# IRMVLab/EfficientLO-Net

Hardware: AMD Instinct MI355X
Metric: frame-pairs/sec (KITTI 64x1800 range image) (higher is better)
Workload: dtype f32 (1x1 convolutions as 3 fp16-MFMA products of hi/lo-split fp32 operands, fp32 accumulate)

## Files before the change

### efficientlo-net_amd/csrc/elo_fused.hip

```cpp
#include "elo_group_device.h"
#include "elo_project_device.h"
#include <atomic>
#include <cstdlib>
#include <type_traits>

namespace elo {
namespace {

typedef float f32x4 __attribute__((ext_vector_type(4)));
typedef _Float16 half4 __attribute__((ext_vector_type(4)));
typedef _Float16 half2v __attribute__((ext_vector_type(2)));

constexpr int FUSED_BLOCK = 256;
constexpr int FUSED_WAVES = 4;
__device__ __forceinline__ int ftid() { return (int)(threadIdx.x & (FUSED_BLOCK - 1)); }

constexpr int MODE_SPLIT = 0;
constexpr int MODE_HALF = 1;
constexpr int MODE_CHECKED = 2;

__device__ unsigned long long g_range_violations;
__device__ unsigned long long g_range_snapshot;
__global__ void range_take_kernel() { g_range_snapshot = atomicExch(&g_range_violations, 0ull); }

// ... 1493 lines not shown
    const int kq = lane >> 4, i16 = lane & 15;
    const long p = first_point + (K == 16 ? r >> 4 : r >> 3);
    const bool writer = (i16 & (K - 1)) == 0 && p < total_points;
#pragma unroll
    for (int cb = 0; cb < NOUT / 16; ++cb) {
        const float q[4] = {last[cb].x * mk, last[cb].y * mk, last[cb].z * mk, last[cb].w * mk};
        float o[4];
#pragma unroll
        for (int e = 0; e < 4; ++e) {
            int v = __float_as_int(q[e]);
            v = dpp_imax_all<0xb1>(v);
            v = dpp_imax_all<0x4e>(v);
            v = dpp_imax_all<0x141>(v);
            if (K == 16) v = dpp_imax_all<0x140>(v);
            o[e] = __int_as_float(v);
        }
        if (writer) feat_store4(out, p * NOUT + cb * 16 + 4 * kq, float4{o[0], o[1], o[2], o[3]}, F16);
    }
}

template <bool F16>
__device__ __forceinline__ void rr_pool_softmax4_inwave(const float4 (&logit)[4], const ActPair &v0, const ActPair &v1, float mk, int r,
                                                        int lane, long first_point, long total_points, void *out)
{
    const int kq = lane >> 4, i16 = lane & 15;
    const long p = first_point + (r >> 2);
    const bool writer = (i16 & 3) == 3 && p < total_points;
    auto shr1 = [](float x) { return __int_as_float(__builtin_amdgcn_update_dpp(0, __float_as_int(x), 0x111, 0xf, 0xf, true)); };
    auto quad_lane = [](float x, auto sel) {
        return __int_as_float(__builtin_amdgcn_update_dpp(0, __float_as_int(x), decltype(sel)::value * 0x55, 0xf, 0xf, true));
    };
    const int j = i16 & 3;
#pragma unroll
    for (int cb = 0; cb < 4; ++cb) {
        const ActPair &xp = cb < 2 ? v0 : v1;
        const float4 val = cb % 2 == 0 ? quad_value(xp.hi.x, xp.hi.y, xp.lo.x, xp.lo.y) : quad_value(xp.hi.z, xp.hi.w, xp.lo.z, xp.lo.w);
        const float l[4] = {logit[cb].x, logit[cb].y, logit[cb].z, logit[cb].w}, v[4] = {val.x, val.y, val.z, val.w};
        float den[4], acc[4];
#pragma unroll
        for (int e = 0; e < 4; ++e) {
            const float x = mk == 1.0f ? l[e] : -1e10f;
            int m = __float_as_int(x);
            m = dpp_imax_all<0xb1>(m);
            m = dpp_imax_all<0x4e>(m);
            const float ex = exp_hw(x - __int_as_float(m)), ev = ex * v[e];
            float cd = ex, ca = ev;
#pragma unroll
            for (int step = 0; step < 3; ++step) { cd = shr1(cd) + ex; ca = shr1(ca) + ev; }
            den[e] = cd; acc[e] = ca;
        }
        typedef std::integral_constant<int, 3> L3;
        float a4[4], d4[4];
#pragma unroll
        for (int e = 0; e < 4; ++e) { a4[e] = quad_lane(acc[e], L3{}); d4[e] = quad_lane(den[e], L3{}); }
        const float aj = j == 0 ? a4[0] : j == 1 ? a4[1] : j == 2 ? a4[2] : a4[3], dj = j == 0 ? d4[0] : j == 1 ? d4[1] : j == 2 ? d4[2] : d4[3];
        const float qj = aj / dj;
        const float4 o{quad_lane(qj, std::integral_constant<int, 0>{}), quad_lane(qj, std::integral_constant<int, 1>{}),
                       quad_lane(qj, std::integral_constant<int, 2>{}), quad_lane(qj, L3{})};
        if (writer) feat_store4(out, p * 64 + cb * 16 + 4 * kq, o, F16);
    }
}

constexpr int RR_BIAS_OFF = 8192;
template <int NL>
__device__ __forceinline__ float rr_bias_request(const float *const (&b)[NL], const int (&n)[NL], int tid)
{
    int at = tid;
    const float *src = b[0];
    bool found = false;
#pragma unroll
    for (int l = 0; l < NL; ++l) {
        if (!found && at < n[l]) { src = b[l] + at; found = true; }
        at -= n[l];
    }
    return *src;
}
__device__ __forceinline__ void rr_bias_store(float *lds, int tid, int total, float v) { if (tid < total) lds[RR_BIAS_OFF + tid] = v; }

template <int FP> struct Cv1Plan {
    static constexpr int NL = 6;
    static constexpr int KP[6] = {FP, 4, 2, 0, 4, 4}, TL[6] = {1, 0, 0, 1, 0, 0}, NCB[6] = {8, 4, 4, 4, 8, 4};
};

template <int C, bool F16, int MODE = MODE_SPLIT>
__device__ __forceinline__ void cv1_rr_body(const elo_cv1_args &a, const unsigned block, const unsigned nblocks)
{
    extern __shared__ __align__(16) float lds[];
    constexpr int FP = C / 16;
    const int lane = threadIdx.x & 63, wave = __builtin_amdgcn_readfirstlane(threadIdx.x >> 6);
    const int i16 = lane & 15, kq = lane >> 4;
    uint4 *ring = reinterpret_cast<uint4 *>(lds);
    const int K = a.K, P = RR_ROWS / K;
    const long total_points = (long)a.batch * a.npoints;
    const long first_point = (long)xcd_tile(block, nblocks) * P;
    unsigned bad = 0;
    RR_STAMP(0);
    typedef RrStream<Cv1Plan<FP>, MODE> Stream;
    Stream ws{{a.cv0.w_packed, a.cv1.w_packed, a.cv2.w_packed, a.cv_xyz.w_packed, a.sum_cv0.w_packed, a.sum_cv1.w_packed}, ring, wave, lane, {}};
    constexpr int E0 = Stream::first(1), E1 = Stream::first(2), E2 = Stream::first(3), E3 = Stream::first(4), E4 = Stream::first(5);
    auto fetch = [&](int g, RrW &dst) { ws.fetch(g, dst); };
    auto advance = [&](int S) { ws.advance(S); };
    ws.start();
    float4 bias[2];
#pragma unroll
    for (int t = 0; t < 2; ++t) bias[t] = *reinterpret_cast<const float4 *>(a.cv0.bias + t * 16 + 4 * kq);
    const float *const bsrc[6] = {a.cv0.bias, a.cv1.bias, a.cv2.bias, a.cv_xyz.bias, a.sum_cv0.bias, a.sum_cv1.bias};
    constexpr int BN[6] = {128, 64, 64, 64, 128, 64}, B1 = 128, B2 = 192, B3 = 256, B4 = 320, B5 = 448;
    const float bias_word = rr_bias_request(bsrc, BN, (int)threadIdx.x);
    const float *bt = lds + RR_BIAS_OFF;
    const int r = wave * 16 + i16, pi = small_div(r, K);
    long pt = first_point + pi;
    const bool used = pi < P && pt < total_points;
    if (!used) pt = first_point;
    const long gr = used ? pt * K + (r - pi * K) : first_point * K;
    const int id0 = a.idx[gr * 3 + 0], id1 = a.idx[gr * 3 + 1], id2 = a.idx[gr * 3 + 2];
    float mk = a.mask[gr];
    const int cell = (id0 * a.H2 + id1) * a.W2 + id2;
    if (!used) mk = 0.0f;
    const bool keep2 = used && mk != 0.0f;
    ActPair in0[FP];
    uint4 geo;
    {
        typedef typename std::conditional<F16, uint2, float4>::type Item;
        Item f1[FP], f2[FP];
        const Item *r1 = reinterpret_cast<const Item *>(a.feat1) + (pt * C >> 2) + kq;
        const Item *r2 = reinterpret_cast<const Item *>(a.feat2) + ((long)cell * C >> 2) + kq;
#pragma unroll
        for (int j = 0; j < FP; ++j) { f1[j] = r1[j * 4]; f2[j] = r2[j * 4]; }
        const float *c = a.xyz1 + pt * 3, *g = a.xyz2 + (long)cell * 3;
        const float pc0 = c[0], pc1 = c[1], pc2 = c[2], pg0 = g[0], pg1 = g[1], pg2 = g[2];
        ws.prime();
        auto quad = [&](const Item &v, bool keep) {
            const uint4 z{0u, 0u, 0u, 0u};
            if constexpr (F16) return keep ? quad_of_halves(v) : z;
            else return keep ? pack_quad<MODE>(v, bad) : z;
        };
#pragma unroll
        for (int j = 0; j < FP; ++j) put_quad(in0[j / 2], j % 2, quad(f1[j], used));
#pragma unroll
        for (int j = 0; j < FP; ++j) put_quad(in0[(FP + j) / 2], (FP + j) % 2, quad(f2[j], keep2));
        const float g0 = pg0 * mk, g1 = pg1 * mk, g2 = pg2 * mk;
        const float d0 = g0 - pc0, d1 = g1 - pc1, d2 = g2 - pc2;
        const float e = sqrtf(d0 * d0 + d1 * d1 + d2 * d2 + 1e-20f);
        const float4 q4 = kq == 0 ? float4{pc0, pc1, pc2, g0} : kq == 1 ? float4{g1, g2, d0, d1}
                        : kq == 2 ? float4{d2, e, 0.0f, 0.0f} : float4{0.0f, 0.0f, 0.0f, 0.0f};
        geo = used ? pack_quad<MODE>(q4, bad) : uint4{0u, 0u, 0u, 0u};
    }
    rr_bias_store(lds, (int)threadIdx.x, 512, bias_word);
    RR_STAMP(1);
    rr_barrier();
    RR_LAYER_STAMP(2);
    const uint4 none{0u, 0u, 0u, 0u};
    ActPair h128[4];
    auto emit0 = [&](int pass, int t, const f32x4 acc) { put_quad(h128[pass], t, pack_quad<MODE>(relu4(acc, a.cv0.relu), bad)); };
    rr_layer<FP, true, 8, 0, MODE, (F16 ? ~0u : 0u)>(in0, geo, bt, bt + B1, bias, fetch, advance, emit0);
    RR_LAYER_STAMP(3);
    ActPair h64[2];
    rr_layer<4, false, 4, E0, MODE>(h128, none, bt + B1, bt + B2, bias, fetch, advance, [&](int pass, int t, const f32x4 acc) {
        put_quad(h64[pass], t, pack_quad<MODE>(relu4(acc, a.cv1.relu), bad));
    });
    RR_LAYER_STAMP(4);
    ActPair xe[4];
    rr_layer<2, false, 4, E1, MODE>(h64, none, bt + B2, bt + B3, bias, fetch, advance, [&](int pass, int t, const f32x4 acc) {
        put_quad(xe[pass], t, pack_quad<MODE>(relu4(acc, a.cv2.relu), bad));
    });
    RR_LAYER_STAMP(5);
    {
        ActPair unused[1];
        rr_layer<0, true, 4, E2, MODE>(unused, geo, bt + B3, bt + B4, bias, fetch, advance, [&](int pass, int t, const f32x4 acc) {
            put_quad(xe[2 + pass], t, pack_quad<MODE>(relu4(acc, a.cv_xyz.relu), bad));
        });
    }
    RR_LAYER_STAMP(6);
    rr_layer<4, false, 8, E3, MODE>(xe, none, bt + B4, bt + B5, bias, fetch, advance, [&](int pass, int t, const f32x4 acc) {
        put_quad(h128[pass], t, pack_quad<MODE>(relu4(acc, a.sum_cv0.relu), bad));
    });
    RR_LAYER_STAMP(7);
    float4 logit[4];
    rr_layer<4, false, 4, E4, MODE>(h128, none, bt + B5, nullptr, bias, fetch, advance, [&](int pass, int t, const f32x4 acc) {
        logit[2 * pass + t] = relu4(acc, a.sum_cv1.relu);
    });
    RR_STAMP(8);
    rr_pool<F16>(lds, logit, xe[0], xe[1], mk, r, wave, lane, K, P, first_point, total_points, a.out);
    RR_STAMP(9);
    report_violations<MODE>(bad, a.range_counter);
}

template <int C, bool F16, int MODE = MODE_SPLIT>
__global__ __launch_bounds__(RR_WAVES * 64, 4) void cv1_rr_kernel(const elo_cv1_args a)
{
    cv1_rr_body<C, F16, MODE>(a, blockIdx.x, gridDim.x);
}
template <int C> struct Cv2Plan {
    static constexpr int NL = 3;
    static constexpr int KP[3] = {0, 4 + C / 32, 4}, TL[3] = {1, C == 16 ? 1 : 0, 0}, NCB[3] = {4, 8, 4};
};

template <int C, bool F16, int MODE = MODE_SPLIT>
__global__ __launch_bounds__(RR_WAVES * 64, 4) void cv2_rr_kernel(const elo_cv2_args a)
{
    extern __shared__ __align__(16) float lds[];
// ... 308 lines not shown
        for (int j = 0; j < 2; ++j) {
            if (!live[j]) continue;
            const int pp = (wave * 16) / K + j, b = pb[j];
            const float cx = pc[j][0], cy = pc[j][1], cz = pc[j][2];
            auto emit = [&](int slot, int hw) {
                cell_row[pp * K + slot] = (b * a.H2 + (hw >> 16)) * a.W2 + (hw & 0xffff);
                mask_row[pp * K + slot] = 1.0f;
            };
            int count = 0;
            if (!(pick_max(sq3(cx, cy, cz), ELO_EPS) <= ELO_EPS)) {
                const GridBuf gb = grid_buffer(a.src_xyz + (size_t)b * a.H2 * a.W2 * 3);
                count = wave_random_k_prefetched(gb, a.H2, a.W2, KT, K, lds_off, ph[j], pw[j], cx, cy, cz, r2, first[j], emit);
            }
            if (count + lane < K) { cell_row[pp * K + count + lane] = 0; mask_row[pp * K + count + lane] = 0.0f; }
        }
    }
    RR_STAMP(2);
    __syncthreads();
    RR_STAMP(3);
    const int r = wave * 16 + i16, pi = small_div(r, K);
    const int cell = cell_row[r];
    const bool used = cell >= 0;
    const float mk = mask_row[r];
    const float c0 = cxyz[(pi < P ? pi : 0) * 3 + 0], c1 = cxyz[(pi < P ? pi : 0) * 3 + 1], c2 = cxyz[(pi < P ? pi : 0) * 3 + 2];
    ActPair in0[FPB / 2];
    uint4 dxyz;
    const bool keep = used && mk != 0.0f;
    {
        typedef typename std::conditional<F16, uint2, float4>::type Item;
        Item f[FPB];
        const long cc = used ? cell : 0;
        const Item *rf = reinterpret_cast<const Item *>(a.src_feat) + (cc * C >> 2) + kq;
#pragma unroll
        for (int j = 0; j < FPB; ++j) f[j] = rf[j * 4];
        const float *g = a.src_xyz + cc * 3;
        const float x = g[0], y = g[1], z = g[2];
        ws.prime();
        auto quad = [&](const Item &v) {
            const uint4 zq{0u, 0u, 0u, 0u};
            if constexpr (F16) return keep ? quad_of_halves(v) : zq;
            else return keep ? pack_quad<MODE>(v, bad) : zq;
        };
#pragma unroll
        for (int j = 0; j < FPB; ++j) put_quad(in0[j / 2], j % 2, quad(f[j]));
        const float4 d = kq == 0 ? float4{x * mk - c0, y * mk - c1, z * mk - c2, 0.0f} : float4{0.0f, 0.0f, 0.0f, 0.0f};
        dxyz = used ? pack_quad<MODE>(d, bad) : uint4{0u, 0u, 0u, 0u};
    }
    rr_bias_store(lds, tid, N1 + N2 + N3, bias_word);
    RR_STAMP(4);
    rr_barrier();
    RR_STAMP(5);
    const uint4 none{0u, 0u, 0u, 0u};
    ActPair h1[N1 / 32];
    auto emit0 = [&](int pass, int t, const f32x4 acc) { put_quad(h1[pass], t, pack_quad<MODE>(relu4(acc, a.layers[0].relu), bad)); };
    rr_layer<FPB / 2, true, N1 / 16, 0, MODE, (F16 ? ~0u : 0u)>(in0, dxyz, bt, bt + B1, bias, fetch, advance, emit0);
    RR_STAMP(6);
    float4 last[NOUT / 16];
    if constexpr (N3 == 0) {
        rr_layer<N1 / 32, false, N2 / 16, E0, MODE>(h1, none, bt + B1, nullptr, bias, fetch, advance, [&](int pass, int t, const f32x4 acc) {
            last[2 * pass + t] = relu4(acc, a.layers[1].relu);
        });
    } else {
        ActPair h2[N2 / 32];
        rr_layer<N1 / 32, false, N2 / 16, E0, MODE>(h1, none, bt + B1, bt + B2, bias, fetch, advance, [&](int pass, int t, const f32x4 acc) {
            put_quad(h2[pass], t, pack_quad<MODE>(relu4(acc, a.layers[1].relu), bad));
        });
        rr_layer<N2 / 32, false, NOUT / 16, E1, MODE>(h2, none, bt + B2, nullptr, bias, fetch, advance, [&](int pass, int t, const f32x4 acc) {
            last[2 * pass + t] = relu4(acc, a.layers[2].relu);
        });
    }
    RR_STAMP(7);
    if ((K == 8 || K == 16) && a.layers[N3 ? 2 : 1].relu) rr_pool_max_inwave<NOUT, F16>(last, mk, r, lane, K, first_point, total_points, a.out);
    else rr_pool_max<NOUT, F16>(lds, last, mk, r, wave, lane, K, P, first_point, total_points, a.out);
    RR_STAMP(8);
    report_violations<MODE>(bad, a.range_counter);
}

template <int FPB, int N1, int N2, int N3, bool F16, int MODE = MODE_SPLIT>
__global__ __launch_bounds__(RR_WAVES * 64, 4) void setconv_rr_kernel(const JobPair<elo_setconv_args> jobs)
{
    setconv_rr_body<FPB, N1, N2, N3, F16, MODE>(jobs.job[blockIdx.y], blockIdx.x, gridDim.x);
}

template <int C, bool F16, int MODE>
__global__ __launch_bounds__(RR_WAVES * 64, 4) void cv1_setconv_rr_kernel(const elo_cv1_args a, const JobPair<elo_setconv_args> jobs,
                                                                         const unsigned n_cv, const unsigned n_sc)
{
    if (blockIdx.x < n_cv) {
        cv1_rr_body<C, F16, MODE>(a, blockIdx.x, n_cv);
    } else {
        const unsigned r = blockIdx.x - n_cv, j = r >= n_sc ? 1u : 0u;
        setconv_rr_body<4, 128, 64, 0, F16, MODE>(jobs.job[j], j ? r - n_sc : r, n_sc);
    }
}
template <int CIN, int N1, int N2, int N3, int MODE>
__global__ __launch_bounds__(ELO_BLOCK, 2) void setconv_narrow_kernel(const elo_setconv_args a)
{
    constexpr int G = 32, PER_BLOCK = ELO_BLOCK / G, C = CIN - 3, CB3 = N3 / 16;
    static_assert((C == 16 || C == 3) && N1 <= 16 && N2 <= 16 && (N3 == 16 || N3 == 32), "the pyramid's two narrow set-conv layers");
    __shared__ int slot_hw[PER_BLOCK][G];
    const int tid = threadIdx.x;
    const int l64 = tid & 63, i16 = l64 & 15, kq = l64 >> 4;
    unsigned bad = 0, wbad = 0;
    auto wq = [&](const elo_dense &L, const int LK, const int LN, int k0, int n) {
        const int nc = n < LN ? n : LN - 1;
        float v[4];
#pragma unroll
        for (int e = 0; e < 4; ++e) {
            const int k = k0 + e < LK ? k0 + e : LK - 1;
            v[e] = L.w_plain[k * LN + nc];
        }
#pragma unroll
        for (int e = 0; e < 4; ++e) v[e] = (k0 + e < LK && n < LN) ? v[e] : 0.0f;
        return float4{v[0], v[1], v[2], v[3]};
    };
    auto bq = [&](const elo_dense &L, const int LN, int n0) {
        float v[4];
#pragma unroll
        for (int e = 0; e < 4; ++e) v[e] = L.bias[n0 + e < LN ? n0 + e : LN - 1];
#pragma unroll
        for (int e = 0; e < 4; ++e) v[e] = n0 + e < LN ? v[e] : 0.0f;
        return float4{v[0], v[1], v[2], v[3]};
    };
    const float4 w1a = wq(a.layers[0], CIN, N1, 4 * kq, i16), w1b = C == 16 ? wq(a.layers[0], CIN, N1, 16 + 4 * kq, i16) : float4{0.0f, 0.0f, 0.0f, 0.0f};
    const float4 w2f = wq(a.layers[1], N1, N2, 4 * kq, i16);
    float4 w3f[CB3];
#pragma unroll
    for (int cb = 0; cb < CB3; ++cb) w3f[cb] = wq(a.layers[2], N2, N3, 4 * kq, cb * 16 + i16);
    const float4 b1 = bq(a.layers[0], N1, 4 * kq), b2 = bq(a.layers[1], N2, 4 * kq);
    float4 b3[CB3];
#pragma unroll
    for (int cb = 0; cb < CB3; ++cb) b3[cb] = bq(a.layers[2], N3, cb * 16 + 4 * kq);

    const int g = tid / G, lane = tid % G, shift = (tid & 63) / G * G;
    const elo_group_spec &gs = a.group;
    const int KT = gs.kernel_h * gs.kernel_w, kW = gs.kernel_w, hh = gs.kernel_h / 2, hw2 = gs.kernel_w / 2;
    int off[SMALL_STEPS];
    const int *order = gs.decoded_hw ? gs.decoded_hw : gs.random_hw;
#pragma unroll
    for (int st = 0; st < SMALL_STEPS; ++st) off[st] = order[st * G + lane < KT ? st * G + lane : 0];
    const long total = (long)a.batch * a.npoints;
    const long first = (long)xcd_tile(blockIdx.x, gridDim.x) * PER_BLOCK;
    const long pt = first + g;
    const bool live = pt < total;
    const long ptc = live ? pt : total - 1;
    int b, n, hc, wc;
    split_point(ptc, a.npoints, b, n);
    if (a.centre_hw) {
        const int2 c2 = reinterpret_cast<const int2 *>(a.centre_hw)[ptc];
        hc = c2.x; wc = c2.y;
    } else { hc = n / a.W; wc = n - hc * a.W; }
    if (!gs.decoded_hw) {
#pragma unroll
        for (int st = 0; st < SMALL_STEPS; ++st) off[st] = ((off[st] / kW - hh) << 16) | ((off[st] % kW - hw2) & 0xffff);
    }
    const float *cp = a.xyz1_grid + (((long)b * a.H + hc) * a.W + wc) * 3;
    const float cx = cp[0], cy = cp[1], cz = cp[2];
    const float *grid2 = a.src_xyz + (size_t)b * a.H2 * a.W2 * 3;
    const int base_h = div_stride(hc, gs.stride_h), base_w = div_stride(wc, gs.stride_w);
    RawSlot raw[SMALL_STEPS];
#pragma unroll
    for (int st = 0; st < SMALL_STEPS; ++st) raw[st] = fetch_slot(grid2, a.H2, a.W2, off[st], base_h, base_w, st * G + lane < KT);
    if (live && lane < 3 && a.new_xyz) a.new_xyz[pt * 3 + lane] = lane == 0 ? cx : lane == 1 ? cy : cz;
    const float r2 = gs.distance * gs.distance;
    slot_hw[g][lane] = -1;
    int taken = 0;
    const bool centre_ok = !(pick_max(sq3(cx, cy, cz), ELO_EPS) <= ELO_EPS);
#pragma unroll
    for (int st = 0; st < SMALL_STEPS; ++st) {
        if (st > 0 && (st * G >= KT || __builtin_amdgcn_ballot_w64(taken < G) == 0)) break;
        const Probe pr = judge(raw[st], cx, cy, cz, r2);
        const bool hit = pr.hit && centre_ok && taken < G;
// ... 790 lines not shown
        const int P = RR_ROWS / a->K;
        const dim3 grid((unsigned)(((long)a->batch * a->npoints + P - 1) / P));
        const size_t lds = RR_LDS_BYTES;
        hipStream_t s = (hipStream_t)stream;
        const bool f16 = a->feat_dtype == ELO_F16;
        static_assert(RR_LDS_BYTES <= 64 * 1024, "dynamic LDS within the default limit");
#define RR(CC)                                                                                                      \
        do {                                                                                                        \
            if (f16 && plan.mode == MODE_HALF) hipLaunchKernelGGL((cv1_rr_kernel<CC, true, MODE_HALF>), grid, dim3(RR_WAVES * 64), lds, s, *a);          \
            else if (f16) hipLaunchKernelGGL((cv1_rr_kernel<CC, true, MODE_SPLIT>), grid, dim3(RR_WAVES * 64), lds, s, *a);          \
            else if (plan.mode == MODE_HALF) hipLaunchKernelGGL((cv1_rr_kernel<CC, false, MODE_HALF>), grid, dim3(RR_WAVES * 64), lds, s, *a);             \
            else hipLaunchKernelGGL((cv1_rr_kernel<CC, false, MODE_SPLIT>), grid, dim3(RR_WAVES * 64), lds, s, *a);             \
        } while (0)
        if (a->C == 16) RR(16);
        else if (a->C == 32) RR(32);
        else RR(64);
#undef RR
        ++g_rr_launches[0];
        return check_launch(who);
    }
#endif
    const dim3 grid((unsigned)plan.units);
    const size_t lds = plan.lds;
    const int S = plan.S;
    hipStream_t s = (hipStream_t)stream;
#define CALL(k) hipLaunchKernelGGL(k, grid, dim3(FUSED_BLOCK), lds, s, *a, S)
    if (a->group.random_hw) ELO_PICK(cv1_kernel, plan.t16, plan.mode, CALL);
    else ELO_PICK(cv1_meta_kernel, plan.t16, plan.mode, CALL);
#undef CALL
    return check_launch(who);
}


extern "C" int elo_cv_stage1_setconv_fused(const elo_cv1_args *a, const elo_setconv_args *ja, const elo_setconv_args *jb,
                                           elo_stream_t stream)
{
    const char *who = "elo_cv_stage1_setconv_fused";
    TilePlan pc, ps;
    if (int rc = plan_cv1(a, &pc, who)) return rc;
    if (int rc = check_setconv(ja, who)) return rc;
    if (jb) {
        if (int rc = check_setconv(jb, who)) return rc;
        if (!same_shape(ja, jb)) return fail(ELO_ERR_ARG, "%s: the two set-conv jobs must have the same shape", who);
    }
    if (int rc = plan_setconv(ja, jb, &ps, who)) return rc;
    if (ps.mode != pc.mode) return fail(ELO_ERR_ARG, "%s: the cost volume and the set-conv jobs must share one products mode", who);
    if ((long)a->batch * a->npoints == 0 || (long)ja->batch * ja->npoints == 0)
        return fail(ELO_ERR_ARG, "%s: empty batch (call the separate entry points)", who);
    SideJobs side;
    side.job[0] = *ja;
    side.job[1] = jb ? *jb : *ja;
    side.njobs = jb ? 2 : 1;
    side.S = ps.S;
    side.blocks_per_job = (int)ps.units;
    const unsigned n_cv = (unsigned)pc.units;
    const dim3 grid(n_cv + (unsigned)(ps.units * side.njobs));
    const size_t lds = pc.lds > ps.lds ? pc.lds : ps.lds;
    const int S = pc.S;
    hipStream_t s = (hipStream_t)stream;
#define CALL_T(M) do {                                                                                                  \
        if (pc.t16 && ps.t16) hipLaunchKernelGGL((cv1_setconv_kernel<16, 16, M>), grid, dim3(FUSED_BLOCK), lds, s, *a, S, n_cv, side);      \
        else if (pc.t16) hipLaunchKernelGGL((cv1_setconv_kernel<16, 32, M>), grid, dim3(FUSED_BLOCK), lds, s, *a, S, n_cv, side);           \
        else if (ps.t16) hipLaunchKernelGGL((cv1_setconv_kernel<32, 16, M>), grid, dim3(FUSED_BLOCK), lds, s, *a, S, n_cv, side);           \
        else hipLaunchKernelGGL((cv1_setconv_kernel<32, 32, M>), grid, dim3(FUSED_BLOCK), lds, s, *a, S, n_cv, side);                        \
    } while (0)
    ELO_PICK_MODE(pc.mode, CALL_T);
#undef CALL_T
    return check_launch(who);
}

static int chain_pair_form(const elo_cv1_args *a, const elo_setconv_args *ja, const elo_setconv_args *jb, int *mode_out, const char *who)
{
#ifdef ELO_DENSE_F32
    (void)a; (void)ja; (void)jb; (void)mode_out; (void)who;
    return 0;
#else
    if (!a || !ja || !jb) return 0;
    int mode = 0, mode_sc = 0, mode_sb = 0;
    if (products_mode(who, &mode, a->cv0, a->cv1, a->cv2, a->cv_xyz, a->sum_cv0, a->sum_cv1)) return 0;
    if (ja->n_layers != 2 || jb->n_layers != 2 || products_mode(who, &mode_sc, ja->layers, 2) || products_mode(who, &mode_sb, jb->layers, 2)) return 0;
    if (mode != mode_sc || mode != mode_sb || !same_shape(ja, jb) || ja->feat_dtype != a->feat_dtype) return 0;
    if (!cv_chain(a->C, mode) || setconv_chain_shape(ja, jb, mode) != 1) return 0;
    if (a->K <= 0 || a->K > 32) return 0;
    *mode_out = mode;
    return 1;
#endif
}

extern "C" int elo_cv_stage1_setconv_chain_form(const elo_cv1_args *a, const elo_setconv_args *ja, const elo_setconv_args *jb)
{
    int mode = 0;
    return chain_pair_form(a, ja, jb, &mode, "elo_cv_stage1_setconv_chain_form");
}

extern "C" int elo_cv_stage1_setconv_chain(const elo_cv1_args *a, const elo_setconv_args *ja, const elo_setconv_args *jb,
                                           elo_stream_t stream)
{
    const char *who = "elo_cv_stage1_setconv_chain";
#ifdef ELO_DENSE_F32
    (void)a; (void)ja; (void)jb; (void)stream;
    return fail(ELO_ERR_LIMIT, "%s: the fp32-MFMA comparison build has no register-resident kernels", who);
#else
    TilePlan pc, ps;
    if (int rc = plan_cv1(a, &pc, who)) return rc;
    ELO_REQUIRE(jb, who, "two set-conv jobs");
    if (int rc = check_setconv(ja, who)) return rc;
    if (int rc = check_setconv(jb, who)) return rc;
    if (!same_shape(ja, jb)) return fail(ELO_ERR_ARG, "%s: the two set-conv jobs must have the same shape", who);
    if (int rc = plan_setconv(ja, jb, &ps, who)) return rc;
    if (a->group.random_hw || !a->idx || !a->mask) return fail(ELO_ERR_ARG, "%s: the cost volume comes pre-grouped (idx / mask of the select-k pre-pass)", who);
    int mode = 0;
    if (!chain_pair_form(a, ja, jb, &mode, who) || mode != pc.mode || mode != ps.mode)
        return fail(ELO_ERR_ARG, "%s: not a chain-form launch (elo_cv_stage1_setconv_chain_form returns 0)", who);
    const long pts_cv = (long)a->batch * a->npoints, pts_sc = (long)ja->batch * ja->npoints;
    if (pts_cv == 0 || pts_sc == 0) return fail(ELO_ERR_ARG, "%s: empty batch (call the separate entry points)", who);
    const int Pc = RR_ROWS / a->K, Ps = RR_ROWS / ja->K;
    const unsigned n_cv = (unsigned)((pts_cv + Pc - 1) / Pc), n_sc = (unsigned)((pts_sc + Ps - 1) / Ps);
    const dim3 grid(n_cv + 2u * n_sc);
    JobPair<elo_setconv_args> pair;
    pair.job[0] = *ja;
    pair.job[1] = *jb;
    hipStream_t s = (hipStream_t)stream;
    const bool f16 = a->feat_dtype == ELO_F16;
#define RRP(CC)                                                                                                                              \
    do {                                                                                                                                    \
        if (f16 && mode == MODE_HALF) hipLaunchKernelGGL((cv1_setconv_rr_kernel<CC, true, MODE_HALF>), grid, dim3(RR_WAVES * 64), RR_LDS_BYTES, s, *a, pair, n_cv, n_sc);   \
        else if (f16) hipLaunchKernelGGL((cv1_setconv_rr_kernel<CC, true, MODE_SPLIT>), grid, dim3(RR_WAVES * 64), RR_LDS_BYTES, s, *a, pair, n_cv, n_sc);                 \
        else if (mode == MODE_HALF) hipLaunchKernelGGL((cv1_setconv_rr_kernel<CC, false, MODE_HALF>), grid, dim3(RR_WAVES * 64), RR_LDS_BYTES, s, *a, pair, n_cv, n_sc);   \
        else hipLaunchKernelGGL((cv1_setconv_rr_kernel<CC, false, MODE_SPLIT>), grid, dim3(RR_WAVES * 64), RR_LDS_BYTES, s, *a, pair, n_cv, n_sc);                          \
    } while (0)
    if (a->C == 16) RRP(16);
    else if (a->C == 32) RRP(32);
    else RRP(64);
#undef RRP
    ++g_rr_launches[0];
    ++g_rr_launches[2];
    ++g_chain_pair_launches;
    return check_launch(who);
#endif
}

static int plan_cv2(const elo_cv2_args *a, TilePlan *p, const char *who)
{
    ELO_REQUIRE(a, who, "null argument block");
    ELO_REQUIRE(a->batch >= 0 && a->npoints > 0 && a->K > 0 && a->H > 0 && a->W > 0 && a->C > 0, who, "bad sizes");
    ELO_REQUIRE(a->npoints == a->H * a->W, who, "npoints must equal H*W (every pixel is a centre)");
    if (a->K > 32) return fail(ELO_ERR_LIMIT, "%s: K = %d exceeds the 32-row tile", who, a->K);
    if (a->C > 64) return fail(ELO_ERR_LIMIT, "%s: C = %d exceeds 64", who, a->C);
    ELO_REQUIRE(a->xyz1 && a->feat1 && a->cost && a->out, who, "null tensor pointer");
    ELO_REQUIRE(a->group.random_hw || (a->idx && a->mask), who, "neither idx/mask nor a grouping spec");
    if (int rc = check_dtype(a->feat_dtype, who)) return rc;
    if (int rc = check_cv_features(who, a->C, a->feat_dtype == ELO_F16, {a->feat1, a->cost})) return rc;
    if (int rc = check_dense(a->xyz_enc, 10, 64, who, "sum_xyz_encoding")) return rc;
    if (int rc = check_dense(a->sum_cost0, 128 + a->C, 128, who, "sum_cost_volume_0")) return rc;
    if (int rc = check_dense(a->sum_cost1, 128, 64, who, "sum_cost_volume_1")) return rc;
    const long points = (long)a->batch * a->npoints;
    if (points >= 0x7fffffffL) return fail(ELO_ERR_LIMIT, "%s: batch * npoints beyond 2^31", who);
    p->units = 0;
    if (points == 0) return ELO_OK;
    p->S = row_stride(208);
    const int P32 = 32 / a->K, P16 = a->K <= 16 ? 16 / a->K : 1;
    const long u32 = (points + P32 - 1) / P32, u16 = (points + P16 - 1) / P16;
    if (int rc = products_mode(who, &p->mode, a->xyz_enc, a->sum_cost0, a->sum_cost1)) return rc;
    p->t16 = small_tile(u32, a->K);
    p->units = p->t16 ? u16 : u32;
    const int KT = a->group.random_hw ? a->group.kernel_h * a->group.kernel_w : 0;
    p->lds = tile_lds_bytes(p->t16 ? 16 : 32, p->S, KT, false);
    return check_group(a->group, a->H, a->W, p->lds, who);
}

extern "C" int elo_cv_stage2_fused(const elo_cv2_args *a, elo_stream_t stream)
{
    const char *who = "elo_cv_stage2_fused";
    TilePlan plan;
    if (int rc = plan_cv2(a, &plan, who)) return rc;
    if (plan.units == 0) return ELO_OK;
    const int S = plan.S, mode = plan.mode;
    const bool t16 = plan.t16;
    const size_t lds = plan.lds;
    hipStream_t s = (hipStream_t)stream;
#ifndef ELO_DENSE_F32
    if (!a->group.random_hw && cv_chain(a->C, mode)) {
        const int P = RR_ROWS / a->K;
        const dim3 rgrid((unsigned)(((long)a->batch * a->npoints + P - 1) / P));
        const bool f16 = a->feat_dtype == ELO_F16;
#define RR(CC)                                                                                                           \
        do {                                                                                                             \
            if (f16 && mode == MODE_HALF) hipLaunchKernelGGL((cv2_rr_kernel<CC, true, MODE_HALF>), rgrid, dim3(RR_WAVES * 64), RR_LDS_BYTES, s, *a);     \
            else if (f16) hipLaunchKernelGGL((cv2_rr_kernel<CC, true, MODE_SPLIT>), rgrid, dim3(RR_WAVES * 64), RR_LDS_BYTES, s, *a);     \
            else if (mode == MODE_HALF) hipLaunchKernelGGL((cv2_rr_kernel<CC, false, MODE_HALF>), rgrid, dim3(RR_WAVES * 64), RR_LDS_BYTES, s, *a);        \
            else hipLaunchKernelGGL((cv2_rr_kernel<CC, false, MODE_SPLIT>), rgrid, dim3(RR_WAVES * 64), RR_LDS_BYTES, s, *a);        \
        } while (0)
        if (a->C == 16) RR(16);
        else if (a->C == 32) RR(32);
        else RR(64);
#undef RR
        ++g_rr_launches[1];
        return check_launch(who);
    }
#endif
    const dim3 grid((unsigned)plan.units);
#define CALL(k) hipLaunchKernelGGL(k, grid, dim3(FUSED_BLOCK), lds, s, *a, S)
    ELO_PICK(cv2_kernel, t16, mode, CALL);
#undef CALL
    return check_launch(who);
}

static int upconv_ride_plan(const elo_cv2_args *a, const elo_mlp_args *ja, const elo_mlp_args *jb, TilePlan *pc, MlpPlan *pm,
                            const char *who)
{
    if (int rc = plan_cv2(a, pc, who)) return rc;
    ELO_REQUIRE(ja && jb, who, "two set-upconv jobs");
    if (int rc = plan_mlp(ja, jb, pm, who)) return rc;
    if (pc->units == 0 || ja->rows == 0) return fail(ELO_ERR_ARG, "%s: empty cost volume or jobs (call the separate entry points)", who);
    for (const elo_mlp_args *j : {ja, jb})
        if (j->n_layers2 != 0 || j->clear_scratch || j->sv_scratch)
// ... 46 lines not shown
```

### efficientlo-net_amd/fused.py

```python
import ctypes
import os

import torch

from . import _lib as L
from . import tf_util, tuning


def fp32_mfma():
    return bool(L.lib().elo_dense_f32())


PRODUCTS_SPLIT, PRODUCTS_HALF = 0, 1
_products = PRODUCTS_SPLIT


def products_mode():
    return _products


class products:

    def __init__(self, mode):
        self.mode = {"split": PRODUCTS_SPLIT, "half": PRODUCTS_HALF, PRODUCTS_SPLIT: PRODUCTS_SPLIT,
# ... 292 lines not shown

def _mlp2_args(sources, layers, before, after, layers2):
    a, out, keep = _mlp_args(sources, layers)
    rows = out.shape[0]
    before, after = _features(before, after, out)[0][:2]
    flat = lambda t: None if t is None else t.reshape(rows, t.shape[-1])
    before, after = flat(before), flat(after)
    out2 = torch.empty((rows, layers2[-1].N), dtype=out.dtype, device=out.device)
    a.n_layers2, a.layers2, a.out2 = len(layers2), _chain(layers2), out2.data_ptr()
    a.before, a.w_before = (before.data_ptr(), before.shape[1]) if before is not None else (None, 0)
    a.after, a.w_after = (after.data_ptr(), after.shape[1]) if after is not None else (None, 0)
    return a, out, out2, (keep, before, after, layers2)


def mlp2_pair(job_a, job_b, clear=None, sv=None):
    a, out_a, out2_a, _ka = _mlp2_args(**job_a)
    b, out_b, out2_b, _kb = _mlp2_args(**job_b)
    if _ride_sv(a, b, sv, out_a.dtype) or sv is None:
        _ride_clear(a, clear, out_a.dtype)
    L.call2("elo_mlp_fused2", a, b, out_a)
    lead = job_a["sources"][0].shape[:-1]
    shape = lambda t: t.reshape(lead + (t.shape[-1],))
    return (shape(out_a), shape(out2_a)), (shape(out_b), shape(out2_b))


THROUGHPUT_BATCH = 4


def _prepass_rows(stage=1, batch=1):
    e = tuning.get("cv_prepass")
    if e is None:
        return 8192 if batch >= THROUGHPUT_BATCH else (20000 if stage == 1 else 65536)
    return (1 << 60) if e == 0 else 0 if e == 1 else int(e)


_HW = {}


def _all_pixels(B, H, W, device):
    key = (B, H, W, str(device))
    hit = _HW.get(key)
    if hit is None:
        hh = torch.arange(H, dtype=torch.int32, device=device).view(1, H, 1, 1).expand(B, H, W, 1)
        ww = torch.arange(W, dtype=torch.int32, device=device).view(1, 1, W, 1).expand(B, H, W, 1)
        hit = torch.cat([hh, ww], -1).reshape(B, H * W, 2).contiguous()
        if hit.is_cuda and torch.cuda.is_current_stream_capturing():
            return hit
        if len(_HW) >= 64:
            _HW.clear()
        _HW[key] = hit
    return hit




def group_prepass(kind, xyz1_grid, xyz2_grid, group, K):
    B, H, W, _ = xyz1_grid.shape
    _, H2, W2, _ = xyz2_grid.shape
    N, kH, kW = H * W, group.kernel_h, group.kernel_w
    idx = torch.empty((B, N, K, 3), dtype=torch.int32, device=xyz1_grid.device)
    mask = torch.empty((B, N, K), dtype=torch.float32, device=xyz1_grid.device)
    if kind == "select":
        from .fused_conv import _select_dense_fits
        dense = -(-W // 64) * H * B >= tuning.get("select_dense_tiles") and _select_dense_fits(kH, kW, K, 0, group.stride_h, group.stride_w)
        entry = "elo_fused_conv_select_k_dense" if dense else "elo_fused_conv_select_k"
    else:
        RH, RW = 1 // group.stride_h + kH, 63 // group.stride_w + kW
        dense = 4 * ((kH * kW + 7) & ~7) + 16 * RH * RW + 4 * (129 * K + 256) <= 64 * 1024
        entry = "elo_fused_conv_random_k_dense" if dense else "elo_fused_conv_random_k"
    hw = None if dense else _all_pixels(B, H, W, xyz1_grid.device)
    a = L.GroupArgs(B, H, W, H2, W2, N, kH, kW, K, 0, group.distance, group.stride_h, group.stride_w,
                    xyz1_grid.data_ptr(), xyz2_grid.data_ptr(), None if dense else hw.data_ptr(), group.random_hw.data_ptr(),
                    idx.data_ptr(), None, None, mask.data_ptr())
    L.call(entry, a, idx)
    return idx, mask


def _rr_path(group, B, N, K, C, stage=1):
    return (group is not None and not group.want_indices and K <= 32 and B * N * K >= _prepass_rows(stage, B)
            and group.stride_h == 1 and group.stride_w == 1 and not fp32_mfma()
            and C in (16, 32, 64))


_RECORD = None


class recording:

    def __enter__(self):
        global _RECORD
        self.prev, _RECORD = _RECORD, []
        return _RECORD

    def __exit__(self, *exc):
        global _RECORD
        _RECORD = self.prev


def _record(stage, args, kwargs):
    keep = lambda v: v.detach().clone() if torch.is_tensor(v) else v
    kw = {k: keep(v) for k, v in kwargs.items() if k != "side"}
    if kwargs.get("group") is not None:
        g = kwargs["group"]
        kw["group"] = Grouping(g.random_hw.clone(), [g.kernel_h, g.kernel_w], g.distance, g.stride_h, g.stride_w)
    _RECORD.append((stage, tuple(keep(v) for v in args), kw, bool(kwargs.get("side"))))


def cv_stage1(xyz1, feat1, xyz2_proj, feat2_proj, idx, mask, cv0, cv1, cv2, cv_xyz, sum_cv0, sum_cv1, group=None, K=None,
              side=None, side_chain=False):
    L.require_gpu(xyz1, feat1, xyz2_proj, feat2_proj, idx, mask)
    if _RECORD is not None:
        _record(1, (xyz1, feat1, xyz2_proj, feat2_proj, idx, mask, cv0, cv1, cv2, cv_xyz, sum_cv0, sum_cv1), dict(group=group, K=K, side=side))
    xyz1, xyz2_proj = _f32c(xyz1), _f32c(xyz2_proj)
    (feat1, feat2_proj), dt, code = _features(feat1, feat2_proj)
    _, H2, W2, C = feat2_proj.shape
    B, N = xyz1.shape[0], xyz1.shape[1]
    ptr = lambda x: x.data_ptr() if x is not None else None
    chain_jobs = None
    if side and side_chain:
        rr = len(side) == 2 and N == H2 * W2 and _rr_path(group, B, N, K, C)
        if rr:
            chain_jobs = [_setconv_args(**job) for job in side]
            probe = L.Cv1Args(B, N, K, H2, W2, C, None, None, None, None, None, None, cv0.struct(), cv1.struct(), cv2.struct(),
                              cv_xyz.struct(), sum_cv0.struct(), sum_cv1.struct(), None, _NO_GROUP, code)
            if L.lib().elo_cv_stage1_setconv_chain_form(ctypes.byref(probe), ctypes.byref(chain_jobs[0][0]), ctypes.byref(chain_jobs[1][0])) != 1:
                chain_jobs = None
        if chain_jobs is None:
            return cv_stage1_alone(xyz1, feat1, xyz2_proj, feat2_proj, idx, mask, cv0, cv1, cv2, cv_xyz, sum_cv0, sum_cv1, group, K), None
    if (not side or chain_jobs) and N == H2 * W2 and _rr_path(group, B, N, K, C):
        idx, mask = group_prepass("select", xyz1.reshape(B, H2, W2, 3), xyz2_proj, group, K)
        group = None
    if group is None:
        idx, mask = idx.contiguous(), _f32c(mask)
        K = idx.shape[2]
    out = torch.empty((B, N, 64), dtype=dt, device=xyz1.device)
    a = L.Cv1Args(B, N, K, H2, W2, C, xyz1.data_ptr(), feat1.data_ptr(), xyz2_proj.data_ptr(), feat2_proj.data_ptr(),
                  ptr(idx), ptr(mask), cv0.struct(), cv1.struct(), cv2.struct(), cv_xyz.struct(),
                  sum_cv0.struct(), sum_cv1.struct(), out.data_ptr(),
                  group.struct(B, N, K, xyz1.device) if group is not None else _NO_GROUP, code)
    if chain_jobs:
        L.call3("elo_cv_stage1_setconv_chain", a, chain_jobs[0][0], chain_jobs[1][0], out)
        return out, [(j[1], j[2]) for j in chain_jobs]
    if side:
        jobs = [_setconv_args(**job) for job in side]
        L.call3("elo_cv_stage1_setconv_fused", a, jobs[0][0], jobs[1][0] if len(jobs) > 1 else None, out)
        return out, [(j[1], j[2]) for j in jobs]
    L.call("elo_cv_stage1_fused", a, out)
    return out


def cv_stage1_alone(xyz1, feat1, xyz2_proj, feat2_proj, idx, mask, cv0, cv1, cv2, cv_xyz, sum_cv0, sum_cv1, group, K):
    global _RECORD
    keep, _RECORD = _RECORD, None
    try:
        return cv_stage1(xyz1, feat1, xyz2_proj, feat2_proj, idx, mask, cv0, cv1, cv2, cv_xyz, sum_cv0, sum_cv1, group=group, K=K)
    finally:
        _RECORD = keep


def cv_stage2(xyz1_proj, feat1_proj, cost_proj, idx, mask, xyz_enc, sum_cost0, sum_cost1, group=None, K=None, side=None):
    L.require_gpu(xyz1_proj, feat1_proj, cost_proj, idx, mask)
    if _RECORD is not None:
        _record(2, (xyz1_proj, feat1_proj, cost_proj, idx, mask, xyz_enc, sum_cost0, sum_cost1), dict(group=group, K=K, side=side))
    xyz1_proj = _f32c(xyz1_proj)
    (feat1_proj, cost_proj), dt, code = _features(feat1_proj, cost_proj)
    B, H, W, C = feat1_proj.shape
    N = H * W
    ptr = lambda x: x.data_ptr() if x is not None else None
    if _rr_path(group, B, N, K, C, stage=2):
        idx, mask = group_prepass("random", xyz1_proj, xyz1_proj, group, K)
        group = None
    if group is None:
        idx, mask = idx.contiguous(), _f32c(mask)
        K = idx.shape[2]
    out = torch.empty((B, N, 64), dtype=dt, device=xyz1_proj.device)
    a = L.Cv2Args(B, N, K, H, W, C, xyz1_proj.data_ptr(), feat1_proj.data_ptr(), cost_proj.data_ptr(), ptr(idx),
                  ptr(mask), xyz_enc.struct(), sum_cost0.struct(), sum_cost1.struct(), out.data_ptr(),
                  group.struct(B, N, K, xyz1_proj.device) if group is not None else _NO_GROUP, code)
    if side:
        if B < THROUGHPUT_BATCH:
            jobs = [_mlp_args(**job) for job in side]
            if L.lib().elo_cv_stage2_upconv_form(ctypes.byref(a), ctypes.byref(jobs[0][0]), ctypes.byref(jobs[1][0])) == 1:
                L.call3("elo_cv_stage2_upconv_fused", a, jobs[0][0], jobs[1][0], out)
                return out, [j[1].reshape(job["sources"][0].shape[:-1] + (j[1].shape[-1],)) for j, job in zip(jobs, side)]
        L.call("elo_cv_stage2_fused", a, out)
        return out, None
    L.call("elo_cv_stage2_fused", a, out)
    return out
```

### efficientlo-net_amd/tuning.py

```python
import contextlib
import hashlib
import json
import os

def _prepass(spec):
    return None if spec in (None, "") else int(spec)


_HOST = {
    "fused": ("ELO_FUSED", lambda v: v != "0", True),
    "cv_prepass": ("ELO_CV_PREPASS", _prepass, None),
    "select_dense_tiles": ("ELO_SELECT_DENSE_TILES", int, 1024),
    "merge_points": ("ELO_MERGE_POINTS", int, 8192),
    "merge_level_points": ("ELO_MERGE_LEVEL_POINTS", int, 2000),
    "chain_pair": ("ELO_CHAIN_PAIR", lambda v: v != "0", True),
    "native_submit": ("ELO_NATIVE_SUBMIT", lambda v: v != "0", True),
    "sv_ride": ("ELO_SV_RIDE", lambda v: v != "0", True),
    "upconv_ride": ("ELO_UPCONV_RIDE", lambda v: v != "0", True),
    "train_kernels": ("ELO_TRAIN_KERNELS", lambda v: v != "0", True),
    "train_dense": ("ELO_TRAIN_DENSE", lambda v: v != "0", True),
    "train_dense_rows": ("ELO_TRAIN_DENSE_ROWS", int, 25000),
    "train_siamese_batch": ("ELO_TRAIN_SIAMESE_BATCH", lambda v: v != "0", True),
    "train_dense_fused_dz": ("ELO_TRAIN_DENSE_FUSED_DZ", lambda v: v != "0", True),
    "train_dense_dx_rows": ("ELO_TRAIN_DENSE_DX_ROWS", int, 100000),
}
_LIB = {
    "chain_forms": ("ELO_CV1_RR", 1), "narrow_mfma": ("ELO_SETCONV_NARROW_MFMA", 1), "range_check": ("ELO_RANGE_CHECK", 0),
    "select_dense_waves": ("ELO_SELECT_DENSE_WAVES", 0), "random_dense_rows": ("ELO_DENSE_ROWS", 0),
    "setconv_chain_rows": ("ELO_SETCONV_RR_ROWS", -1), "mlp_chain_rows": ("ELO_MLP_RR_ROWS", -1), "small_tile_units": ("ELO_SMALL_TILE_UNITS", 64),
    "pool_wave": ("ELO_POOL_WAVE", 1),
}


_LIB_BOOLEAN = ("chain_forms", "narrow_mfma", "range_check", "pool_wave")


def _host_from_env():
    out = {}
    for name, (var, parse, default) in _HOST.items():
        raw = os.environ.get(var)
        out[name] = default if raw is None else parse(raw)
    return out


def lib_from_env():
    out = {}
    for name, (var, _default) in _LIB.items():
        raw = os.environ.get(var)
        if raw is not None:
            value = int(raw)
            out[name] = (1 if value else 0) if name in _LIB_BOOLEAN else value
    return out


_host = _host_from_env()
_version = 0


def version():
    return _version


def bump():
    global _version
    _version += 1


def get(name):
    return _host[name]


def set_host(name, value):
    if name not in _HOST:
        raise KeyError(name)
    prev, _host[name] = _host[name], value
    bump()
    return prev


@contextlib.contextmanager
def override(**fields):
    from . import _lib
    host = {k: v for k, v in fields.items() if k in _HOST}
    lib = {k: v for k, v in fields.items() if k in _LIB}
    unknown = set(fields) - set(host) - set(lib)
    if unknown:
        raise KeyError("unknown tuning field(s): %s" % sorted(unknown))
    prev_host = {k: _host[k] for k in host}
    prev_lib = _lib.get_tuning_base() if lib else None
    try:
        _host.update(host)
        bump()
        if lib:
            _lib.set_tuning(**lib)
        yield
    finally:
        _host.update(prev_host)
        bump()
        if prev_lib is not None:
            _lib.set_tuning(**prev_lib)
# ... 17 lines not shown
```

Baseline: 12670.

## Fuse select-k grouping into the cost-volume chain kernel instead of a pre-pass

Adds an in-kernel select-k grouping stage to the cv1 chain kernel. Each block computes neighbor cells and masks into LDS scratch rather than reading idx/mask written by a separate group pre-pass kernel. This drops one kernel launch and the global round trip of idx/mask. In exchange it adds a barrier and serial per-wave selection work at the start of each cost-volume block, which may lengthen the kernel or raise register/LDS pressure.

```diff
diff --git a/efficientlo-net_amd/csrc/elo_cv1_rr_group.h b/efficientlo-net_amd/csrc/elo_cv1_rr_group.h
--- /dev/null
+++ b/efficientlo-net_amd/csrc/elo_cv1_rr_group.h
@@ -0,0 +1,57 @@
+#pragma once
+
+constexpr int CV1_RR_GROUP_OFF = 4096;
+static_assert(CV1_RR_GROUP_OFF + ((512 + 3) & ~3) + 6 * RR_ROWS + RR_WAVES * 128 <= RR_BIAS_OFF, "select-k scratch in front of the bias table");
+
+__device__ __forceinline__ void cv1_rr_group(const elo_cv1_args &a, float *lds, int P, int K, long first_point, long total_points,
+                                             int wave, int lane)
+{
+    const int tid = threadIdx.x;
+    const int KT = a.group.kernel_h * a.group.kernel_w;
+    int *lds_off = reinterpret_cast<int *>(lds + CV1_RR_GROUP_OFF);
+    int *cell_row = lds_off + ((KT + 3) & ~3);
+    float *mask_row = reinterpret_cast<float *>(cell_row + RR_ROWS);
+    int *chw = reinterpret_cast<int *>(mask_row + RR_ROWS);
+    float *cxyz = reinterpret_cast<float *>(chw + RR_ROWS);
+    unsigned *scratch = reinterpret_cast<unsigned *>(cxyz + 3 * RR_ROWS);
+    if (tid < RR_ROWS) { cell_row[tid] = -1; mask_row[tid] = 0.0f; }
+    if (tid < P) {
+        const long pt = first_point + tid;
+        const long pq = pt < total_points ? pt : first_point;
+        const int b = (int)((unsigned)pq / (unsigned)a.npoints), n = (int)((unsigned)pq - (unsigned)b * (unsigned)a.npoints);
+        const int hc = n / a.W2, wc = n - hc * a.W2;
+        const float *c = a.xyz1 + (((long)b * a.H2 + hc) * a.W2 + wc) * 3;
+        const float cx = c[0], cy = c[1], cz = c[2];
+        if (pt < total_points) { chw[tid] = (hc << 16) | wc; cxyz[tid * 3 + 0] = cx; cxyz[tid * 3 + 1] = cy; cxyz[tid * 3 + 2] = cz; }
+    }
+    stage_offsets(lds_off, a.group.random_hw, a.group.kernel_h, a.group.kernel_w, a.group.decoded_hw);
+    const float r2 = a.group.distance * a.group.distance;
+    auto uniform = [](float v) { return __int_as_float(__builtin_amdgcn_readfirstlane(__float_as_int(v))); };
+    for (int pi = wave; pi < P; pi += RR_WAVES) {
+        const long pt = first_point + pi;
+        if (pt >= total_points) break;
+        const int b = (int)((unsigned)pt / (unsigned)a.npoints);
+        const int hwc = __builtin_amdgcn_readfirstlane(chw[pi]), hc = hwc >> 16, wc = hwc & 0xffff;
+        const float cx = uniform(cxyz[pi * 3 + 0]), cy = uniform(cxyz[pi * 3 + 1]), cz = uniform(cxyz[pi * 3 + 2]);
+        auto emit = [&](int slot, int hw) {
+            cell_row[pi * K + slot] = (b * a.H2 + (hw >> 16)) * a.W2 + (hw & 0xffff);
+            mask_row[pi * K + slot] = 1.0f;
+        };
+        int count = 0;
+        if (!(pick_max(sq3(cx, cy, cz), ELO_EPS) <= ELO_EPS)) {
+            const GridBuf gb = grid_buffer(a.xyz2 + (size_t)b * a.H2 * a.W2 * 3);
+            unsigned *mine = scratch + (size_t)wave * 128;
+            count = wave_select_k(gb, a.H2, a.W2, KT, K, lds_off, div_stride(hc, a.group.stride_h), div_stride(wc, a.group.stride_w),
+                                  cx, cy, cz, r2, mine, reinterpret_cast<int *>(mine) + KT, emit);
+        }
+        for (int k = count + lane; k < K; k += 64) { cell_row[pi * K + k] = 0; mask_row[pi * K + k] = 0.0f; }
+    }
+    rr_barrier();
+}
+
+static bool cv1_rr_select_ok(const elo_cv1_args *a)
+{
+    const int KT = a->group.kernel_h * a->group.kernel_w;
+    return a->group.random_hw && !a->group.idx_out && !a->group.mask_out && a->npoints == a->H2 * a->W2 && KT > 0 && KT <= 512 &&
+           select_in_registers(KT, a->K) && a->group.stride_h > 0 && a->group.stride_w > 0;
+}
diff --git a/efficientlo-net_amd/csrc/elo_fused.hip b/efficientlo-net_amd/csrc/elo_fused.hip
--- a/efficientlo-net_amd/csrc/elo_fused.hip
+++ b/efficientlo-net_amd/csrc/elo_fused.hip
@@ -1599,7 +1599,9 @@
     static constexpr int KP[6] = {FP, 4, 2, 0, 4, 4}, TL[6] = {1, 0, 0, 1, 0, 0}, NCB[6] = {8, 4, 4, 4, 8, 4};
 };
 
-template <int C, bool F16, int MODE = MODE_SPLIT>
+#include "elo_cv1_rr_group.h"
+
+template <int C, bool F16, int MODE = MODE_SPLIT, bool GROUP = false>
 __device__ __forceinline__ void cv1_rr_body(const elo_cv1_args &a, const unsigned block, const unsigned nblocks)
 {
     extern __shared__ __align__(16) float lds[];
@@ -1629,11 +1631,19 @@
     long pt = first_point + pi;
     const bool used = pi < P && pt < total_points;
     if (!used) pt = first_point;
-    const long gr = used ? pt * K + (r - pi * K) : first_point * K;
-    const int id0 = a.idx[gr * 3 + 0], id1 = a.idx[gr * 3 + 1], id2 = a.idx[gr * 3 + 2];
-    float mk = a.mask[gr];
-    const int cell = (id0 * a.H2 + id1) * a.W2 + id2;
-    if (!used) mk = 0.0f;
+    int cell; float mk;
+    if constexpr (GROUP) {
+        cv1_rr_group(a, lds, P, K, first_point, total_points, wave, lane);
+        const int *cell_row = reinterpret_cast<const int *>(lds + CV1_RR_GROUP_OFF) + ((a.group.kernel_h * a.group.kernel_w + 3) & ~3);
+        cell = used ? cell_row[r] : 0;
+        mk = used ? reinterpret_cast<const float *>(cell_row + RR_ROWS)[r] : 0.0f;
+    } else {
+        const long gr = used ? pt * K + (r - pi * K) : first_point * K;
+        const int id0 = a.idx[gr * 3 + 0], id1 = a.idx[gr * 3 + 1], id2 = a.idx[gr * 3 + 2];
+        mk = a.mask[gr];
+        cell = (id0 * a.H2 + id1) * a.W2 + id2;
+        if (!used) mk = 0.0f;
+    }
     const bool keep2 = used && mk != 0.0f;
     ActPair in0[FP];
     uint4 geo;
@@ -2108,12 +2118,12 @@
     setconv_rr_body<FPB, N1, N2, N3, F16, MODE>(jobs.job[blockIdx.y], blockIdx.x, gridDim.x);
 }
 
-template <int C, bool F16, int MODE>
+template <int C, bool F16, int MODE, bool GROUP = false>
 __global__ __launch_bounds__(RR_WAVES * 64, 4) void cv1_setconv_rr_kernel(const elo_cv1_args a, const JobPair<elo_setconv_args> jobs,
                                                                          const unsigned n_cv, const unsigned n_sc)
 {
     if (blockIdx.x < n_cv) {
-        cv1_rr_body<C, F16, MODE>(a, blockIdx.x, n_cv);
+        cv1_rr_body<C, F16, MODE, GROUP>(a, blockIdx.x, n_cv);
     } else {
         const unsigned r = blockIdx.x - n_cv, j = r >= n_sc ? 1u : 0u;
         setconv_rr_body<4, 128, 64, 0, F16, MODE>(jobs.job[j], j ? r - n_sc : r, n_sc);
@@ -3070,6 +3080,7 @@
     if (mode != mode_sc || mode != mode_sb || !same_shape(ja, jb) || ja->feat_dtype != a->feat_dtype) return 0;
     if (!cv_chain(a->C, mode) || setconv_chain_shape(ja, jb, mode) != 1) return 0;
     if (a->K <= 0 || a->K > 32) return 0;
+    if (a->group.random_hw && !cv1_rr_select_ok(a)) return 0;
     *mode_out = mode;
     return 1;
 #endif
@@ -3096,7 +3107,9 @@
     if (int rc = check_setconv(jb, who)) return rc;
     if (!same_shape(ja, jb)) return fail(ELO_ERR_ARG, "%s: the two set-conv jobs must have the same shape", who);
     if (int rc = plan_setconv(ja, jb, &ps, who)) return rc;
-    if (a->group.random_hw || !a->idx || !a->mask) return fail(ELO_ERR_ARG, "%s: the cost volume comes pre-grouped (idx / mask of the select-k pre-pass)", who);
+    const bool group = a->group.random_hw != nullptr;
+    if (group ? !cv1_rr_select_ok(a) : (!a->idx || !a->mask))
+        return fail(ELO_ERR_ARG, "%s: neither idx / mask of the select-k pre-pass nor a grouping spec the in-kernel select-k takes", who);
     int mode = 0;
     if (!chain_pair_form(a, ja, jb, &mode, who) || mode != pc.mode || mode != ps.mode)
         return fail(ELO_ERR_ARG, "%s: not a chain-form launch (elo_cv_stage1_setconv_chain_form returns 0)", who);
@@ -3110,16 +3123,15 @@
     pair.job[1] = *jb;
     hipStream_t s = (hipStream_t)stream;
     const bool f16 = a->feat_dtype == ELO_F16;
-#define RRP(CC)                                                                                                                              \
+#define RRP(CC, G)                                                                                                                           \
     do {                                                                                                                                    \
-        if (f16 && mode == MODE_HALF) hipLaunchKernelGGL((cv1_setconv_rr_kernel<CC, true, MODE_HALF>), grid, dim3(RR_WAVES * 64), RR_LDS_BYTES, s, *a, pair, n_cv, n_sc);   \
-        else if (f16) hipLaunchKernelGGL((cv1_setconv_rr_kernel<CC, true, MODE_SPLIT>), grid, dim3(RR_WAVES * 64), RR_LDS_BYTES, s, *a, pair, n_cv, n_sc);                 \
-        else if (mode == MODE_HALF) hipLaunchKernelGGL((cv1_setconv_rr_kernel<CC, false, MODE_HALF>), grid, dim3(RR_WAVES * 64), RR_LDS_BYTES, s, *a, pair, n_cv, n_sc);   \
-        else hipLaunchKernelGGL((cv1_setconv_rr_kernel<CC, false, MODE_SPLIT>), grid, dim3(RR_WAVES * 64), RR_LDS_BYTES, s, *a, pair, n_cv, n_sc);                          \
+        if (f16 && mode == MODE_HALF) hipLaunchKernelGGL((cv1_setconv_rr_kernel<CC, true, MODE_HALF, G>), grid, dim3(RR_WAVES * 64), RR_LDS_BYTES, s, *a, pair, n_cv, n_sc);   \
+        else if (f16) hipLaunchKernelGGL((cv1_setconv_rr_kernel<CC, true, MODE_SPLIT, G>), grid, dim3(RR_WAVES * 64), RR_LDS_BYTES, s, *a, pair, n_cv, n_sc);                 \
+        else if (mode == MODE_HALF) hipLaunchKernelGGL((cv1_setconv_rr_kernel<CC, false, MODE_HALF, G>), grid, dim3(RR_WAVES * 64), RR_LDS_BYTES, s, *a, pair, n_cv, n_sc);   \
+        else hipLaunchKernelGGL((cv1_setconv_rr_kernel<CC, false, MODE_SPLIT, G>), grid, dim3(RR_WAVES * 64), RR_LDS_BYTES, s, *a, pair, n_cv, n_sc);                          \
     } while (0)
-    if (a->C == 16) RRP(16);
-    else if (a->C == 32) RRP(32);
-    else RRP(64);
+    if (a->C == 16) { if (group) RRP(16, true); else RRP(16, false); } else if (a->C == 32) { if (group) RRP(32, true); else RRP(32, false); }
+    else { if (group) RRP(64, true); else RRP(64, false); }
 #undef RRP
     ++g_rr_launches[0];
     ++g_rr_launches[2];
diff --git a/efficientlo-net_amd/fused.py b/efficientlo-net_amd/fused.py
--- a/efficientlo-net_amd/fused.py
+++ b/efficientlo-net_amd/fused.py
@@ -398,6 +398,11 @@
             and C in (16, 32, 64))
 
 
+def _rr_select(group, K):
+    KT = group.kernel_h * group.kernel_w
+    return bool(tuning.get("cv_rr_select")) and KT <= 512 and (K <= 8 or (KT <= 192 and K <= 32))
+
+
 _RECORD = None
 
 
@@ -443,7 +448,7 @@
                 chain_jobs = None
         if chain_jobs is None:
             return cv_stage1_alone(xyz1, feat1, xyz2_proj, feat2_proj, idx, mask, cv0, cv1, cv2, cv_xyz, sum_cv0, sum_cv1, group, K), None
-    if (not side or chain_jobs) and N == H2 * W2 and _rr_path(group, B, N, K, C):
+    if (not side or chain_jobs) and N == H2 * W2 and _rr_path(group, B, N, K, C) and not (chain_jobs and _rr_select(group, K)):
         idx, mask = group_prepass("select", xyz1.reshape(B, H2, W2, 3), xyz2_proj, group, K)
         group = None
     if group is None:
diff --git a/efficientlo-net_amd/tuning.py b/efficientlo-net_amd/tuning.py
--- a/efficientlo-net_amd/tuning.py
+++ b/efficientlo-net_amd/tuning.py
@@ -16,6 +16,7 @@
     "chain_pair": ("ELO_CHAIN_PAIR", lambda v: v != "0", True),
     "native_submit": ("ELO_NATIVE_SUBMIT", lambda v: v != "0", True),
     "sv_ride": ("ELO_SV_RIDE", lambda v: v != "0", True),
+    "cv_rr_select": ("ELO_CV_RR_SELECT", lambda v: v != "0", True),
     "upconv_ride": ("ELO_UPCONV_RIDE", lambda v: v != "0", True),
     "train_kernels": ("ELO_TRAIN_KERNELS", lambda v: v != "0", True),
     "train_dense": ("ELO_TRAIN_DENSE", lambda v: v != "0", True),
```

After: 12580 (median of 2 runs). Within noise of the previous version (-0.7%).
